# pengsongyou/openscene

Measured on NVIDIA B200. Metric: voxels/s MinkUNet34C fwd + 768-d cosine-sim, higher is better.
Workload: dtype bf16x3 (split fp32 operands, fp32 accumulate)

## Files before the change

### include/osb200.h

```cpp
#ifndef OSB200_H
#define OSB200_H

#include <stddef.h>
#include <stdint.h>

#ifdef __cplusplus
extern "C" {
#endif

#define OSB_VERSION 100

int         osb_version(void);
const char *osb_last_error(void);
int osb_device_info(int *sm_count, int *cc_major, int *cc_minor);
int64_t osb_launch_count(void);
int osb_measure_sm_mhz(float *mhz_dev, void *stream);

size_t osb_coordset_workspace_bytes(int64_t n);

int osb_coordset_build(const int32_t *coords, int64_t n, int32_t *coords_int, int32_t *perm, int32_t *inv_perm,
                       void *slots, int64_t cap, int32_t *status_host, void *ws, size_t ws_bytes, void *stream);

int osb_coordset_stride(const int32_t *coords_fine, int64_t n, int32_t new_ts, int32_t *coords_coarse,
                        int32_t *parent_of, int64_t *n_coarse_host, void *ws, size_t ws_bytes, void *stream);
// ... 6 lines not shown

int osb_kernel_map_build(const int32_t *coords_out, int64_t n_out, const void *slots_in, int64_t cap_in,
                         int32_t ks_x, int32_t ks_y, int32_t ks_z, int32_t step, int32_t *nbr,
                         int32_t *pairs_per_k, void *stream);

int osb_kernel_map_transpose(const int32_t *nbr, int64_t n_out, int32_t K, int32_t *nbr_t, int64_t n_in,
                             void *stream);

int osb_conv_fwd_f32(const float *in, int64_t ld_in, const int32_t *nbr, int64_t n_out, int32_t K,
                     const float *w, int32_t cin, int32_t cout, int32_t transpose_w, float *out, void *stream);

int osb_conv_wgrad_f32(const float *in, const int32_t *nbr, int64_t n_out, int32_t K, const float *gout,
                       int32_t cin, int32_t cout, float *gw, void *stream);

size_t osb_conv_wgrad_tc_workspace_bytes(int64_t n_out, int32_t K, int32_t cin, int32_t cout);
int osb_conv_wgrad_tc(const void *x_split, int32_t cin, int64_t n_in, const int32_t *nbr, int64_t n_out, int32_t K,
                      const void *gout_split, int32_t cout, float *gw, void *ws, size_t ws_bytes, void *stream);

size_t osb_conv_packed_weight_bytes(int32_t K, int32_t cin, int32_t cout);
size_t osb_conv_tc_workspace_bytes(int64_t n_out, int32_t K, int32_t cin, int32_t cout);
int osb_conv_pack_weights(const float *w, int32_t K, int32_t cin, int32_t cout, int32_t transpose_w,
                          void *wpack, void *stream);
int osb_conv_fwd_tc(const void *src0, int32_t c0, int64_t n_src0, const void *src1, int32_t c1, int64_t n_src1,
                    const int32_t *nbr, int64_t n_out, int32_t K, const void *wpack, int32_t cout,
                    const float *scale, const float *shift, const void *res, int32_t relu, void *out_split,
                    float *out_f32, const int32_t *out_row_map, void *ws, size_t ws_bytes, int32_t flags, void *stream);

int osb_convtr_fwd_tc(const void *src, int32_t cin, int64_t n_coarse, const int32_t *down_nbr, int32_t kvol, const void *wpack,
                      int32_t cout, const float *scale, const float *shift, int32_t relu, void *out_split, float *out_f32,
                      int32_t flags, void *stream);


size_t osb_conv_desc_bytes(void);
size_t osb_conv_weight_tiles_bytes(int32_t K, int32_t cin, int32_t cout);
int osb_conv_pack_weight_tiles(const float *w, int32_t K, int32_t cin, int32_t cout, int32_t transpose_w, void *wtiles,
                               void *stream);
int osb_conv_chain_grid(void);
size_t osb_conv_chain_workspace_bytes(int64_t n_out, int32_t K, int32_t cin, int32_t cout);
int osb_conv_desc_fill(void *desc_host, const void *src0, int32_t c0, const void *src1, int32_t c1, const int32_t *nbr,
                       int64_t n_out, int32_t K, const void *wtiles, int32_t cout, const float *scale, const float *shift,
                       const void *res, int32_t relu, void *out_split, float *out_f32, const int32_t *out_row_map,
                       const int32_t *cmap, int32_t cmap_cout, void *ws, size_t ws_bytes, int32_t barrier_before);
int osb_conv_chain_launch(const void *descs_host, int32_t n_layers, void *grid_barrier, int32_t flags, void *stream);

int osb_tuning_set(const char *name, int64_t value);

int osb_conv_stem_fused(const float *in, int32_t cin, const int32_t *coords, int64_t n, const void *slots,
                        int64_t cap, int32_t ks, int32_t step, const float *w, int32_t cout, const float *scale,
                        const float *shift, int32_t relu, void *out_split, float *out_f32, void *stream);

int osb_f32_to_split(const float *in, int64_t n, int32_t c, void *out_split, void *stream);
int osb_split_to_f32(const void *in_split, int64_t n, int32_t c, float *out, void *stream);

int osb_gather_rows_f32(const float *in, const int32_t *idx, int64_t n_out, int32_t c, float *out, void *stream);

int osb_match_scores(const void *feat, int32_t feat_is_f16, int64_t n_vox, int32_t c, const int64_t *inds_reverse,
                     int64_t n_pts, const void *text_f16, int32_t k_text, int32_t normalize, void *scores_f16,
                     int64_t *label, float *smax, void *stream);
int osb_match_ensemble(const float *feat3d, const void *feat2d_f16, int64_t n_vox, int32_t c,
                       const int64_t *inds_reverse, int64_t n_pts, const float *smax3d, const float *smax2d,
                       const void *text_f16, int32_t k_text, void *scores_f16, int64_t *label, void *feat_out_f16,
                       void *stream);

int osb_match_accumulate(const void *feat, int32_t feat_is_f16, const void *feat2_f16, const float *sel_a, const float *sel_b,
                         int64_t n_vox, int32_t c, const int64_t *inds_reverse, int64_t n_pts, const void *text_f16,
                         int32_t k_text, int32_t normalize, void *store_f16, int32_t first, int64_t *label, void *stream);
// ... 43 lines not shown
```

### openscene_b200/_cabi.py

```python
import ctypes
import os
from ctypes import c_char_p, c_double, c_int, c_int32, c_int64, c_size_t, c_void_p, POINTER

_HERE = os.path.dirname(os.path.abspath(__file__))
LIB_PATH = os.path.join(_HERE, 'libosb200.so')
_lib = None

P = c_void_p
I32, I64, SZ = c_int32, c_int64, c_size_t

SIGNATURES = {
    'osb_version': (c_int, []),
    'osb_last_error': (c_char_p, []),
    'osb_device_info': (c_int, [POINTER(c_int), POINTER(c_int), POINTER(c_int)]),
    'osb_launch_count': (I64, []),
    'osb_measure_sm_mhz': (c_int, [P, P]),
    'osb_coordset_workspace_bytes': (SZ, [I64]),
    'osb_coordset_build': (c_int, [P, I64, P, P, P, P, I64, POINTER(I32), P, SZ, P]),
    'osb_coordset_stride': (c_int, [P, I64, I32, P, P, POINTER(I64), P, SZ, P]),
    'osb_coordset_pyramid': (c_int, [P, I64, I32, P, P, P, P, I64, P, P, POINTER(I64), POINTER(I32), P, SZ, P]),
    'osb_hash_build': (c_int, [P, I64, P, I64, P]),
    'osb_kernel_map_build': (c_int, [P, I64, P, I64, I32, I32, I32, I32, P, P, P]),
    'osb_kernel_map_transpose': (c_int, [P, I64, I32, P, I64, P]),
    'osb_conv_fwd_f32': (c_int, [P, I64, P, I64, I32, P, I32, I32, I32, P, P]),
    'osb_conv_wgrad_f32': (c_int, [P, P, I64, I32, P, I32, I32, P, P]),
    'osb_conv_wgrad_tc_workspace_bytes': (SZ, [I64, I32, I32, I32]),
    'osb_conv_wgrad_tc': (c_int, [P, I32, I64, P, I64, I32, P, I32, P, P, SZ, P]),
    'osb_conv_packed_weight_bytes': (SZ, [I32, I32, I32]),
    'osb_conv_pack_weights': (c_int, [P, I32, I32, I32, I32, P, P]),
    'osb_conv_tc_workspace_bytes': (SZ, [I64, I32, I32, I32]),
    'osb_conv_fwd_tc': (c_int, [P, I32, I64, P, I32, I64, P, I64, I32, P, I32, P, P, P, I32, P, P, P, P, SZ, I32, P]),
    'osb_convtr_fwd_tc': (c_int, [P, I32, I64, P, I32, P, I32, P, P, I32, P, P, I32, P]),
    'osb_conv_desc_bytes': (SZ, []),
    'osb_conv_weight_tiles_bytes': (SZ, [I32, I32, I32]),
    'osb_conv_pack_weight_tiles': (c_int, [P, I32, I32, I32, I32, P, P]),
    'osb_conv_chain_grid': (c_int, []),
    'osb_conv_chain_workspace_bytes': (SZ, [I64, I32, I32, I32]),
    'osb_conv_desc_fill': (c_int, [P, P, I32, P, I32, P, I64, I32, P, I32, P, P, P, I32, P, P, P, P, I32, P, SZ, I32]),
    'osb_conv_chain_launch': (c_int, [P, I32, P, I32, P]),
    'osb_tuning_set': (c_int, [c_char_p, I64]),
    'osb_conv_stem_fused': (c_int, [P, I32, P, I64, P, I64, I32, I32, P, I32, P, P, I32, P, P, P]),
    'osb_f32_to_split': (c_int, [P, I64, I32, P, P]),
    'osb_split_to_f32': (c_int, [P, I64, I32, P, P]),
    'osb_gather_rows_f32': (c_int, [P, P, I64, I32, P, P]),
    'osb_match_scores': (c_int, [P, I32, I64, I32, P, I64, P, I32, I32, P, P, P, P]),
    'osb_match_ensemble': (c_int, [P, P, I64, I32, P, I64, P, P, P, I32, P, P, P, P]),
    'osb_match_accumulate': (c_int, [P, I32, P, P, P, I64, I32, P, I64, P, I32, I32, P, I32, P, P]),
    'osb_logits_accumulate': (c_int, [P, I64, I32, P, I64, P, I32, P, P, P]),
    'osb_folded_head_finish': (c_int, [P, I64, I32, I32, I32, P, P, P, P]),
    'osb_voxelize_workspace_bytes': (SZ, [I64]),
    'osb_voxelize': (c_int, [P, I32, I64, POINTER(c_double), P, P, P, POINTER(I64), POINTER(c_double), P, SZ, P]),
    'osb_occgrid_bytes': (SZ, [I32, I32]),
    'osb_occgrid_build': (c_int, [P, I64, I32, I32, I32, P, P, P]),
    'osb_kernel_map_build_grid': (c_int, [P, I64, P, I32, I32, I32, I32, I32, I32, I32, P, P, P]),
    'osb_conv_stem_fused_grid': (c_int, [P, I32, P, I64, P, I32, I32, I32, I32, I32, P, I32, P, P, I32, P, P, P]),
    'osb_fusion_workspace_bytes': (SZ, [I64, I32]),
    'osb_fusion_accumulate': (c_int, [P, I32, I64, P, P, P, P, I32, I32, I32, I32, I32, c_double, P, P, P, P, SZ, P]),
    'osb_fusion_finalize': (c_int, [P, P, I64, I32, P, P]),
    'osb_feature_remap_workspace_bytes': (SZ, [I64, I64]),
    'osb_feature_remap': (c_int, [P, I64, P, I64, P, I64, I32, I32, P, P, POINTER(I64), P, SZ, P]),
    'osb_confusion_accumulate': (c_int, [P, P, I32, I64, I32, I32, I32, P, P, P]),
    'osb_intersection_union': (c_int, [P, P, I32, I64, I32, I32, P, P]),
}


def lib():
# ... 41 lines not shown
```

### openscene_b200/csrc/conv_chain.cu

```cuda
#include "tc_ptx.cuh"
#include <algorithm>
#include <cstring>
#include <string>

namespace osb {

constexpr int CH_THREADS = 384;
constexpr int CH_M = 128;
constexpr int CH_A_BYTES = CH_M * 128;
constexpr int CH_STG_BYTES = 4 * 4096;
constexpr int CH_SS_FLOATS = 768;
constexpr int CH_MAX_SA = 12, CH_MAX_SB = 4;
constexpr int CH_W_EPI = 0;
constexpr int CH_W_B = 4;
constexpr int CH_W_MMA = 5;
constexpr int CH_W_A = 7;
constexpr int CH_A_WARPS = 5;
constexpr int CH_DESC_WORDS = 48;
constexpr int CH_MAX_LAYERS = 16;

struct __align__(16) ConvDesc {
  const uint8_t *src0, *src1;
  const int32_t *nbr;
  const uint8_t *wtiles;
  const float *scale, *shift;
  const uint8_t *res;
  uint8_t *out_split;
  float *out_f32;
  const int32_t *out_row_map;
  const int32_t *cmap;
  float *partial;
  int64_t n_out;
  int K, nb0, nb1;
  int cout, cout_pad, nt, n_ntiles;
  int relu, cmap_cout, nsplit, m_tiles;
  int nsub_max;
  int barrier_before;
  int stages_per_split;
  int pad[8];
};
static_assert(sizeof(ConvDesc) == CH_DESC_WORDS * 4, "ConvDesc layout");
struct ChainArgs { ConvDesc d[CH_MAX_LAYERS]; };

__device__ __forceinline__ void bulk_g2s(uint32_t dst, const void *src, uint32_t bytes, uint32_t bar) {
  asm volatile("cp.async.bulk.shared::cluster.global.mbarrier::complete_tx::bytes [%0], [%1], %2, [%3];"
               ::"r"(dst), "l"(src), "r"(bytes), "r"(bar) : "memory");
}
__device__ __forceinline__ void mbar_arrive(uint32_t bar) {
  asm volatile("mbarrier.arrive.shared::cta.b64 _, [%0];" ::"r"(bar) : "memory");
}
__device__ __forceinline__ uint32_t mbar_try(uint32_t bar, uint32_t parity) {
  uint32_t done;
  asm volatile(
      "{\n\t.reg .pred p;\n\t"
      "mbarrier.try_wait.parity.shared::cta.b64 p, [%1], %2;\n\t"
      "selp.u32 %0, 1, 0, p;\n\t}"
      : "=r"(done)
      : "r"(bar), "r"(parity)
      : "memory");
  return done;
}

__device__ long long *g_chain_report = nullptr;
__device__ __noinline__ void chain_stuck(uint32_t bar, uint32_t parity, int tag, uint32_t it) {
  long long *r = g_chain_report;
  if (r && it == (1u << 20) + 1) {
    long long *o = r + 1 + 4 * ((blockIdx.x * 16 + (threadIdx.x >> 5)) % 1024);
    o[0] = ((long long)blockIdx.x << 32) | (threadIdx.x >> 5); o[1] = bar; o[2] = parity; o[3] = tag;
    r[0] = 1;
    __threadfence_system();
  }
  if (it > (1u << 23) || !r) __trap();
}
__device__ __forceinline__ void chain_wait(uint32_t bar, uint32_t parity, int tag) {
  for (uint32_t it = 0;; ++it) {
// ... 15 lines not shown
    if (!done) {
      __nanosleep(sleep_ns);
      if (it > (1u << 24)) __trap();
    }
  }
}
__device__ __forceinline__ unsigned ld_acquire_u32(const unsigned *p) {
  unsigned v;
  asm volatile("ld.acquire.gpu.global.u32 %0, [%1];" : "=r"(v) : "l"(p) : "memory");
  return v;
}

__device__ __forceinline__ void grid_barrier(unsigned *gbar, unsigned &gen) {
  __syncthreads();
  if (threadIdx.x == 0) {
    __threadfence();
    const unsigned old = atomicAdd(gbar, 1u);
    if (old == gridDim.x - 1) {
      gbar[0] = 0;
      __threadfence();
      atomicAdd(gbar + 1, 1u);
    } else {
      unsigned it = 0;
      while (ld_acquire_u32(gbar + 1) == gen) {
        if (++it > (1u << 24)) __trap();
      }
    }
    __threadfence();
  }
  gen += 1;
  __syncthreads();
}

#define CH_PROF_BEGIN() const long long _t0 = prof ? clock64() : 0
#define CH_PROF_END(var) do { if (prof) var += clock64() - _t0; } while (0)

#define CH_KEEP(x) asm volatile("" : "+r"(x))

__device__ __forceinline__ void cp_async16_zfill(uint32_t dst, const void *src, uint32_t ignore) {
  asm volatile(
      "{\n\t.reg .pred p;\n\t"
      "setp.ne.b32 p, %2, 0;\n\t"
      "cp.async.cg.shared.global [%0], [%1], 16, p;\n\t}"
      ::"r"(dst), "l"(src), "r"(ignore)
      : "memory");
}

__global__ void __launch_bounds__(CH_THREADS, 1)
k_conv_chain(const __grid_constant__ ChainArgs args, int n_layers, unsigned *gbar, int sa, int sb, int bslot, int flags,
             long long *dbg_clock) {
  extern __shared__ uint8_t smem_raw[];
  const uint32_t raw_u32 = smem_u32(smem_raw);
  const uint32_t base_u32 = (raw_u32 + 1023u) & ~1023u;
  uint8_t *smem = smem_raw + (base_u32 - raw_u32);
  const uint32_t a_ring = base_u32;
  const uint32_t b_ring = a_ring + (uint32_t)sa * CH_A_BYTES;
  const uint32_t stg_u32 = b_ring + (uint32_t)sb * (uint32_t)bslot;
  uint32_t a_ring_k = a_ring, b_ring_k = b_ring;
  CH_KEEP(a_ring_k); CH_KEEP(b_ring_k);
  uint8_t *aux = smem + (stg_u32 - base_u32) + CH_STG_BYTES;
  float *s_ss = reinterpret_cast<float *>(aux);
  uint64_t *bars = reinterpret_cast<uint64_t *>(s_ss + 2 * CH_SS_FLOATS);
  uint32_t *s_misc = reinterpret_cast<uint32_t *>(bars + 40);

  const int tid = threadIdx.x, warp = tid >> 5, lane = tid & 31;
  if (flags & 1) asm volatile("griddepcontrol.launch_dependents;" ::: "memory");
  const bool prof = dbg_clock != nullptr;
  long long pw0 = 0, pw1 = 0, pw2 = 0, pt = 0;
  if (dbg_clock && tid == 0) dbg_clock[blockIdx.x * 32 + 0] = clock64();
  uint32_t fullA = smem_u32(bars), emptyA = fullA + 12 * 8, fullB = fullA + 24 * 8, emptyB = fullA + 28 * 8;
  uint32_t accFull = fullA + 32 * 8, accEmpty = fullA + 34 * 8;
  CH_KEEP(fullA); CH_KEEP(emptyA); CH_KEEP(fullB); CH_KEEP(emptyB); CH_KEEP(accFull); CH_KEEP(accEmpty);

  if (tid == 0) {
    for (int s = 0; s < sa; ++s) { mbar_init(fullA + 8 * s, 32); mbar_init(emptyA + 8 * s, 1); }
    for (int s = 0; s < sb; ++s) { mbar_init(fullB + 8 * s, 1); mbar_init(emptyB + 8 * s, 2); }
    for (int b = 0; b < 2; ++b) { mbar_init(accFull + 8 * b, 2); mbar_init(accEmpty + 8 * b, 4); }
    asm volatile("fence.mbarrier_init.release.cluster;" ::: "memory");
  }
  if (warp == CH_W_MMA) {
    asm volatile("tcgen05.alloc.cta_group::1.sync.aligned.shared::cta.b32 [%0], %1;" ::"r"(smem_u32(&s_misc[0])), "r"(512u));
    asm volatile("tcgen05.relinquish_alloc_permit.cta_group::1.sync.aligned;");
  }
  unsigned bar_gen = 0;
  if (tid == 0 && gbar) bar_gen = ld_acquire_u32(gbar + 1);
  asm volatile("tcgen05.fence::before_thread_sync;" ::: "memory");
  __syncthreads();
  asm volatile("tcgen05.fence::after_thread_sync;" ::: "memory");
  if (flags & 1) asm volatile("griddepcontrol.wait;" ::: "memory");
  const uint32_t tmem_base = s_misc[0];
  if (dbg_clock && tid == 0) dbg_clock[blockIdx.x * 32 + 1] = clock64();

  uint32_t a_slot = 0, a_phase = 0, b_slot = 0, b_phase = 0, n_item = 0;
  uint32_t g_slot = 0;
  uint32_t p_sl = warp >= CH_W_A ? (uint32_t)(warp - CH_W_A) : 0u, p_lapb = 0, p_par = 0;

  for (int L = 0; L < n_layers; ++L) {
    __syncthreads();
    const ConvDesc *s_desc = &args.d[L];
    const int d_K = s_desc->K, d_nb0 = s_desc->nb0, d_nb1 = s_desc->nb1, d_nt = s_desc->nt, d_n_ntiles = s_desc->n_ntiles;
    const int d_m_tiles = s_desc->m_tiles, d_nsplit = s_desc->nsplit, d_nsub_max = s_desc->nsub_max, d_sps = s_desc->stages_per_split;
    const int64_t d_n_out = s_desc->n_out;
    {
      const int nss = s_desc->cmap ? s_desc->cmap_cout : s_desc->cout;
      const float *sc = s_desc->scale, *sh = s_desc->shift;
      for (int c = tid; c < nss && c < CH_SS_FLOATS; c += CH_THREADS) {
        s_ss[c] = sc ? __ldg(sc + c) : 1.f;
        s_ss[CH_SS_FLOATS + c] = sh ? __ldg(sh + c) : 0.f;
      }
    }
    if (s_desc->barrier_before) {
      grid_barrier(gbar, bar_gen);
    } else {
      __syncthreads();
    }

    const int nb = d_nb0 + d_nb1;
    const int T = d_K * nb;
    const int64_t U = (int64_t)d_m_tiles * d_n_ntiles * d_nsplit;
    const int64_t u_begin = U * blockIdx.x / gridDim.x, u_end = U * (blockIdx.x + 1) / gridDim.x;
    const int per_z = d_m_tiles * d_n_ntiles;
    const uint32_t b_bytes = (uint32_t)d_nt * 128u;

#define CH_FOR_ITEMS()                                                                                         \
    for (int64_t u = u_begin, _n; u < u_end; u += _n)                                                          \
      if (const int z = (int)(u / per_z), r_ = (int)(u - (int64_t)z * per_z), nti = r_ / d_m_tiles,            \
          m = r_ - nti * d_m_tiles, nsub = (d_nsub_max == 2 && u + 1 < u_end && m + 1 < d_m_tiles) ? 2 : 1,    \
          t_begin = min(z * d_sps, T), t_end = min(t_begin + d_sps, T);                                        \
          (_n = nsub, true))

    const long long _role_t0 = prof ? clock64() : 0;
    if (warp == CH_W_B) {
      const uint8_t *wtiles = s_desc->wtiles;
      CH_FOR_ITEMS() {
        (void)m;
        for (int t = t_begin; t < t_end; ++t) {
          { CH_PROF_BEGIN(); mbar_wait_relaxed(emptyB + 8 * b_slot, b_phase ^ 1, 64); CH_PROF_END(pw0); }
          if (elect_one()) {
            const uint32_t fb = fullB + 8 * b_slot;
            if (flags & 0x200) {
              mbar_expect_tx(fb, 0u);
            } else {
              mbar_expect_tx(fb, b_bytes);
              bulk_g2s(b_ring_k + b_slot * (uint32_t)bslot, wtiles + ((int64_t)t * d_n_ntiles + nti) * b_bytes, b_bytes, fb);
            }
          }
          __syncwarp();
          if (++b_slot == (uint32_t)sb) { b_slot = 0; b_phase ^= 1; }
        }
      }
    } else if (warp == CH_W_MMA || warp == CH_W_MMA + 1) {
      const int mi = warp - CH_W_MMA;
      const uint32_t idesc = (1u << 4) | (1u << 7) | (1u << 10) | ((uint32_t)(d_nt >> 3) << 17) | ((uint32_t)(CH_M >> 4) << 24);
      CH_FOR_ITEMS() {
        (void)m; (void)nti;
        const uint32_t buf = n_item & 1u;
        const bool mine = mi < nsub;
        { CH_PROF_BEGIN(); mbar_wait(accEmpty + 8 * buf, ((n_item >> 1) & 1u) ^ 1u); CH_PROF_END(pw2); }
        asm volatile("tcgen05.fence::after_thread_sync;" ::: "memory");
        const uint32_t dcol = tmem_base + buf * 256u + (uint32_t)mi * 128u;
        for (int t = t_begin; t < t_end;) {
          const int nst = min(2, t_end - t);
          uint32_t sl[2], sph[2], bs[2], bph[2];
          {
            uint32_t as_ = a_slot + (uint32_t)mi, ap_ = a_phase, bs_ = b_slot, bp_ = b_phase;
            if (as_ >= (uint32_t)sa) { as_ -= (uint32_t)sa; ap_ ^= 1u; }
// ... 233 lines not shown
            }
            if (d_out_split) {
#pragma unroll
              for (int g = 0; g < 4; ++g) {
                __align__(16) __nv_bfloat16 hh[8], ll[8];
#pragma unroll
                for (int jj = 0; jj < 8; ++jj) split_bf16(y[g * 8 + jj], hh[jj], ll[jj]);
                sts128(my_line + ((g ^ sw) << 4), *reinterpret_cast<const uint4 *>(hh));
                sts128(my_line + (((4 + g) ^ sw) << 4), *reinterpret_cast<const uint4 *>(ll));
              }
              __syncwarp();
              flush_tile(d_out_split, (int64_t)out_c * 4, (int64_t)(oc0 >> 5) * 128, d_cmap != nullptr);
              __syncwarp();
            }
            if (d_out_f32) {
#pragma unroll
              for (int g = 0; g < 8; ++g)
                sts128(my_line + ((g ^ sw) << 4), make_uint4(__float_as_uint(y[4 * g]), __float_as_uint(y[4 * g + 1]),
                                                             __float_as_uint(y[4 * g + 2]), __float_as_uint(y[4 * g + 3])));
              __syncwarp();
              flush_tile(reinterpret_cast<uint8_t *>(d_out_f32), (int64_t)out_c * 4, (int64_t)oc0 * 4,
                         d_row_map != nullptr || d_cmap != nullptr);
              __syncwarp();
            }
          }
        }
        asm volatile("tcgen05.fence::before_thread_sync;" ::: "memory");
        __syncwarp();
        if (lane == 0) mbar_arrive(accEmpty + 8 * buf);
        ++n_item;
      }
    }
#undef CH_FOR_ITEMS
    if (prof) pt += clock64() - _role_t0;

    if (d_nsplit > 1) {
      grid_barrier(gbar, bar_gen);
      const ConvDesc &d = args.d[L];
      const int groups = d.cout / 8;
      const int64_t total = d.n_out * groups;
      for (int64_t e = (int64_t)blockIdx.x * CH_THREADS + tid; e < total; e += (int64_t)gridDim.x * CH_THREADS) {
        const int64_t o = e / groups;
        const int c0 = (int)(e - o * groups) * 8;
        float y[8] = {0.f, 0.f, 0.f, 0.f, 0.f, 0.f, 0.f, 0.f};
        for (int z = 0; z < d.nsplit; ++z) {
          const float4 *pp = reinterpret_cast<const float4 *>(d.partial + ((int64_t)z * d.n_out + o) * d.cout_pad + c0);
          const float4 a = __ldcg(pp), b = __ldcg(pp + 1);
          y[0] += a.x; y[1] += a.y; y[2] += a.z; y[3] += a.w; y[4] += b.x; y[5] += b.y; y[6] += b.z; y[7] += b.w;
        }
        if (d.scale) {
#pragma unroll
          for (int jj = 0; jj < 8; ++jj) y[jj] = fmaf(y[jj], s_ss[c0 + jj], s_ss[CH_SS_FLOATS + c0 + jj]);
        }
        const int64_t off = o * (int64_t)d.cout * 4 + split_off_hi(c0);
        if (d.res) {
          const uint4 hq = __ldcg(reinterpret_cast<const uint4 *>(d.res + off)), lq = __ldcg(reinterpret_cast<const uint4 *>(d.res + off + 64));
          const __nv_bfloat16 *hh = reinterpret_cast<const __nv_bfloat16 *>(&hq);
          const __nv_bfloat16 *ll = reinterpret_cast<const __nv_bfloat16 *>(&lq);
#pragma unroll
          for (int jj = 0; jj < 8; ++jj) y[jj] += join_bf16(hh[jj], ll[jj]);
        }
        if (d.relu) {
#pragma unroll
          for (int jj = 0; jj < 8; ++jj) y[jj] = fmaxf(y[jj], 0.f);
        }
        if (d.out_split) {
          __align__(16) __nv_bfloat16 hh[8], ll[8];
#pragma unroll
          for (int jj = 0; jj < 8; ++jj) split_bf16(y[jj], hh[jj], ll[jj]);
          *reinterpret_cast<uint4 *>(d.out_split + off) = *reinterpret_cast<const uint4 *>(hh);
          *reinterpret_cast<uint4 *>(d.out_split + off + 64) = *reinterpret_cast<const uint4 *>(ll);
        }
        if (d.out_f32) {
          const int64_t orow = d.out_row_map ? (int64_t)__ldg(d.out_row_map + o) : o;
          float4 *op = reinterpret_cast<float4 *>(d.out_f32 + orow * d.cout + c0);
          op[0] = make_float4(y[0], y[1], y[2], y[3]);
          op[1] = make_float4(y[4], y[5], y[6], y[7]);
        }
      }
    }
  }

  if (dbg_clock && tid == 0) dbg_clock[blockIdx.x * 32 + 2] = clock64();
  if (dbg_clock && lane == 0 && (warp == CH_W_B || warp == CH_W_MMA || warp == CH_W_MMA + 1 || warp == CH_W_A || warp == 0)) {
    const int base = warp == CH_W_B ? 4 : warp == CH_W_MMA ? 8 : warp == CH_W_MMA + 1 ? 12 : warp == CH_W_A ? 16 : 20;
    long long *o = dbg_clock + blockIdx.x * 32 + base;
    o[0] = pw0; o[1] = pw1; o[2] = pw2; o[3] = pt;
  }
  asm volatile("tcgen05.fence::before_thread_sync;" ::: "memory");
  __syncthreads();
  if (warp == CH_W_MMA) asm volatile("tcgen05.dealloc.cta_group::1.sync.aligned.b32 %0, %1;" ::"r"(tmem_base), "r"(512u));
}

__global__ void k_pack_weight_tiles(const float *__restrict__ w, int K, int cin, int cout, int cout_pad, int nt, int transpose_w,
                                    uint8_t *__restrict__ wt) {
  const int nb = cin / 32, n_ntiles = cout_pad / nt;
  const int64_t total = (int64_t)K * cout_pad * cin;
  for (int64_t e = (int64_t)blockIdx.x * blockDim.x + threadIdx.x; e < total; e += (int64_t)gridDim.x * blockDim.x) {
    const int c = (int)(e % cin);
    const int64_t kn = e / cin;
    const int ng = (int)(kn % cout_pad), k = (int)(kn / cout_pad);
    float v = 0.f;
    if (ng < cout) v = transpose_w ? w[((int64_t)k * cout + ng) * cin + c] : w[((int64_t)k * cin + c) * cout + ng];
    __nv_bfloat16 hi, lo;
    split_bf16(v, hi, lo);
    const int cb = c >> 5, ci = c & 31, nti = ng / nt, n = ng - nti * nt;
    uint8_t *tile = wt + ((((int64_t)k * nb + cb) * n_ntiles) + nti) * (int64_t)nt * 128;
    const int jh = ci >> 3, el = ci & 7;
    *reinterpret_cast<__nv_bfloat16 *>(tile + n * 128 + (((jh) ^ (n & 7)) << 4) + el * 2) = hi;
    *reinterpret_cast<__nv_bfloat16 *>(tile + n * 128 + (((4 + jh) ^ (n & 7)) << 4) + el * 2) = lo;
  }
}

}

namespace osb { bool conv_tc_tuning(const char *name, int64_t v); }
using namespace osb;

static inline int chain_cout_pad(int cout) { return cout <= 256 ? (cout + 15) / 16 * 16 : (cout + 255) / 256 * 256; }
static inline int chain_nt(int cout) { const int cp = chain_cout_pad(cout); return cp <= 256 ? cp : 256; }

extern "C" {

size_t osb_conv_desc_bytes(void) { return sizeof(ConvDesc); }

size_t osb_conv_weight_tiles_bytes(int32_t K, int32_t cin, int32_t cout) { return (size_t)K * chain_cout_pad(cout) * cin * 4; }

int osb_conv_pack_weight_tiles(const float *w, int32_t K, int32_t cin, int32_t cout, int32_t transpose_w, void *wtiles, void *stream_) {
  cudaStream_t stream = (cudaStream_t)stream_;
  OSB_CHECK(K >= 1 && cin % 32 == 0 && cin > 0 && cout > 0, "osb_conv_pack_weight_tiles: cin (%d) must be a multiple of 32", cin);
  const int cp = chain_cout_pad(cout), nt = chain_nt(cout);
  const int64_t total = (int64_t)K * cp * cin;
  const unsigned grid = (unsigned)std::min<int64_t>(ceil_div(total, 256), 148 * 32);
  k_pack_weight_tiles<<<grid, 256, 0, stream>>>(w, K, cin, cout, cp, nt, transpose_w, (uint8_t *)wtiles);
  OSB_LAUNCH_CHECK();
  return 0;
}

static int chain_nsplit(int64_t n_out, int K, int cin, int cout, int grid_ctas, int force, int nsub_knob) {
  const int cp = chain_cout_pad(cout), nt = chain_nt(cout);
  const int64_t tiles = ceil_div(n_out, CH_M) * (cp / nt);
  const int T = K * (cin / 32);
  const int cap = std::max(1, std::min(32, T));
  if (force > 0) return std::min(force, cap);
  const bool pairs = nt <= 128 && nsub_knob >= 2;
  const int base = (int)std::max<int64_t>(1, std::min<int64_t>(grid_ctas / tiles, cap));
  auto cost = [&](int ns, bool &ok) {
    const int sps = (T + ns - 1) / ns;
    ok = (T + sps - 1) / sps == ns;
    const int64_t upc = ceil_div(tiles * ns, (int64_t)grid_ctas);
    const double per = pairs ? (double)(upc / 2) * 0.75 + (double)(upc % 2) * 0.6 : (double)upc * 0.6 * 1.6;
    double us = per * sps + 4.0;
    if (ns > 1) {
      const double partial_bytes = (double)ns * (double)n_out * cp * 4.0;
      if (partial_bytes > 64e6) ok = false;
      us += 10.0 + 2.0 * partial_bytes / 5e6;
    }
    return us;
  };
  bool ok = true;
  double best = cost(base, ok);
  int best_ns = base;
  for (int ns = base + 1; ns <= cap; ++ns) {
    const double us = cost(ns, ok);
    if (ok && us < best - std::max(0.5, 0.08 * best)) { best = us; best_ns = ns; }
  }
  return best_ns;
}

static int g_chain_force_split = 0;
static int g_chain_nsub = 2;
static int g_chain_grid = 0;
static int g_chain_sa = 0, g_chain_sb = 0;
static long long *g_chain_dbg_clock = nullptr;
static int g_chain_dbg_skip = 0;

int osb_tuning_set(const char *name, int64_t value) {
  const std::string n(name ? name : "");
  if (n == "chain_force_split") g_chain_force_split = (int)value;
  else if (n == "chain_nsub") g_chain_nsub = (int)value;
  else if (n == "chain_grid") g_chain_grid = (int)value;
  else if (n == "chain_sa") g_chain_sa = (int)value;
  else if (n == "chain_sb") g_chain_sb = (int)value;
  else if (n == "chain_dbg_clock") g_chain_dbg_clock = (long long *)(intptr_t)value;
  else if (n == "chain_dbg_skip") g_chain_dbg_skip = (int)value;
  else if (n == "chain_report") {
    long long *ptr = (long long *)(intptr_t)value;
    OSB_CUDA(cudaMemcpyToSymbol(g_chain_report, &ptr, sizeof(ptr)));
  }
  else { OSB_CHECK(conv_tc_tuning(n.c_str(), value), "osb_tuning_set: unknown knob '%s'", n.c_str()); }
  return 0;
}

int osb_conv_chain_grid(void) {
  if (g_chain_grid > 0) return g_chain_grid;
  int dev = 0, sms = 148;
  if (cudaGetDevice(&dev) == cudaSuccess) cudaDeviceGetAttribute(&sms, cudaDevAttrMultiProcessorCount, dev);
  return sms;
}

size_t osb_conv_chain_workspace_bytes(int64_t n_out, int32_t K, int32_t cin, int32_t cout) {
  if (n_out <= 0 || K < 1 || cin < 32 || cout <= 0) return 0;
  const int ns = chain_nsplit(n_out, K, cin, cout, osb_conv_chain_grid(), g_chain_force_split, g_chain_nsub);
  return ns > 1 ? (size_t)ns * n_out * chain_cout_pad(cout) * sizeof(float) : 0;
}

int osb_conv_desc_fill(void *desc_host, const void *src0, int32_t c0, const void *src1, int32_t c1, const int32_t *nbr, int64_t n_out,
                       int32_t K, const void *wtiles, int32_t cout, const float *scale, const float *shift, const void *res,
                       int32_t relu, void *out_split, float *out_f32, const int32_t *out_row_map, const int32_t *cmap,
                       int32_t cmap_cout, void *ws, size_t ws_bytes, int32_t barrier_before) {
  OSB_CHECK(desc_host != nullptr, "osb_conv_desc_fill: no descriptor");
  OSB_CHECK(src0 && c0 > 0 && c0 % 32 == 0 && c1 >= 0 && c1 % 32 == 0, "osb_conv_desc_fill: channel counts must be multiples of 32 (c0=%d c1=%d)", c0, c1);
  OSB_CHECK((c1 == 0) == (src1 == nullptr), "osb_conv_desc_fill: src1 / c1 mismatch");
  OSB_CHECK(K >= 1 && K <= 32, "osb_conv_desc_fill: K=%d not supported (<= 32)", K);
  OSB_CHECK(nbr != nullptr || K == 1, "osb_conv_desc_fill: identity map needs K == 1");
  OSB_CHECK(n_out > 0 && n_out < (1ll << 31), "osb_conv_desc_fill: bad row count");
  OSB_CHECK(cout % 32 == 0 && cout > 0, "osb_conv_desc_fill: cout (%d) must be a multiple of 32", cout);
// ... 1 lines not shown
  OSB_CHECK((scale == nullptr) == (shift == nullptr), "osb_conv_desc_fill: scale and shift go together");
  OSB_CHECK(cmap == nullptr || (cmap_cout > 0 && cmap_cout % 32 == 0 && cout % cmap_cout == 0 && res == nullptr),
            "osb_conv_desc_fill: bad dense-transpose arguments");
  OSB_CHECK((cmap ? cmap_cout : cout) <= CH_SS_FLOATS, "osb_conv_desc_fill: more than %d output channels per row", CH_SS_FLOATS);
  ConvDesc d{};
  const int cin = c0 + c1;
  d.src0 = (const uint8_t *)src0; d.src1 = (const uint8_t *)src1; d.nbr = nbr; d.wtiles = (const uint8_t *)wtiles;
  d.scale = scale; d.shift = shift; d.res = (const uint8_t *)res; d.out_split = (uint8_t *)out_split; d.out_f32 = out_f32;
  d.out_row_map = out_row_map; d.cmap = cmap; d.n_out = n_out; d.K = K; d.nb0 = c0 / 32; d.nb1 = c1 / 32;
  d.cout = cout; d.cout_pad = chain_cout_pad(cout); d.nt = chain_nt(cout); d.n_ntiles = d.cout_pad / d.nt;
  d.relu = relu; d.cmap_cout = cmap_cout; d.m_tiles = (int)ceil_div(n_out, CH_M);
  d.nsub_max = (d.nt <= 128 && g_chain_nsub >= 2) ? 2 : 1;
  d.barrier_before = barrier_before ? 1 : 0;
  d.nsplit = cmap ? 1 : chain_nsplit(n_out, K, cin, cout, osb_conv_chain_grid(), g_chain_force_split, g_chain_nsub);
  const int T = K * (cin / 32);
  d.stages_per_split = (T + d.nsplit - 1) / d.nsplit;
  d.nsplit = (T + d.stages_per_split - 1) / d.stages_per_split;
  d.partial = nullptr;
  if (d.nsplit > 1) {
    const size_t need = (size_t)d.nsplit * n_out * d.cout_pad * sizeof(float);
    OSB_CHECK(ws != nullptr && ws_bytes >= need, "osb_conv_desc_fill: workspace of %zu bytes required (got %zu)", need, ws_bytes);
    d.partial = (float *)ws;
  }
  memcpy(desc_host, &d, sizeof(d));
  return 0;
}

int osb_conv_chain_launch(const void *descs_host, int32_t n_layers, void *grid_barrier_dev, int32_t flags, void *stream_) {
  cudaStream_t stream = (cudaStream_t)stream_;
  OSB_CHECK(descs_host && n_layers >= 1, "osb_conv_chain_launch: bad arguments");
  const ConvDesc *h = (const ConvDesc *)descs_host;
  for (int i = 0; i < n_layers; ++i) {
    OSB_CHECK(i > 0 || !h[i].barrier_before, "osb_conv_chain_launch: the first layer of a launch cannot ask for a barrier");
    OSB_CHECK(i == 0 || h[i].barrier_before || h[i].nsplit == 1 || h[i - 1].nsplit == 1 || h[i].partial != h[i - 1].partial,
              "osb_conv_chain_launch: layers %d and %d share a split workspace without a barrier between them", i - 1, i);
  }
  OSB_SMEM_ATTR_ONCE(k_conv_chain, 227 * 1024);
  const int grid = osb_conv_chain_grid();
  for (int l0 = 0; l0 < n_layers; l0 += CH_MAX_LAYERS) {
    const int cnt = std::min(CH_MAX_LAYERS, n_layers - l0);
    ChainArgs args;
    memcpy(args.d, h + l0, sizeof(ConvDesc) * cnt);
    args.d[0].barrier_before = 0;
    int nt_max = 0, need_bar = 0;
    for (int i = 0; i < cnt; ++i) {
      nt_max = std::max(nt_max, args.d[i].nt);
      need_bar |= (args.d[i].barrier_before || args.d[i].nsplit > 1);
    }
    OSB_CHECK(!need_bar || grid_barrier_dev != nullptr, "osb_conv_chain_launch: this chain needs the grid-barrier words");
    const int bslot = nt_max * 128;
    const int fixed = 1024 + CH_STG_BYTES + 2 * CH_SS_FLOATS * 4 + 40 * 8 + 64;
    int sb = g_chain_sb > 0 ? g_chain_sb : (bslot >= 32768 ? 2 : 3);
    sb = std::min(sb, CH_MAX_SB);
    int sa = (227 * 1024 - fixed - sb * bslot) / CH_A_BYTES;
    if (g_chain_sa > 0) sa = std::min(sa, g_chain_sa);
    sa = std::min(sa, CH_MAX_SA);
    sa &= ~1;
    OSB_CHECK(sa >= 4, "osb_conv_chain_launch: shared memory does not hold four row slots");
    const size_t smem_bytes = (size_t)sa * CH_A_BYTES + (size_t)sb * bslot + fixed;
    cudaLaunchAttribute attr[1];
    attr[0].id = cudaLaunchAttributeProgrammaticStreamSerialization;
    attr[0].val.programmaticStreamSerializationAllowed = 1;
    cudaLaunchConfig_t cfg{};
    cfg.gridDim = dim3((unsigned)grid); cfg.blockDim = dim3(CH_THREADS); cfg.dynamicSmemBytes = smem_bytes; cfg.stream = stream;
    cfg.attrs = attr; cfg.numAttrs = (flags & 1) ? 1 : 0;
    OSB_CUDA(cudaLaunchKernelEx(&cfg, k_conv_chain, args, (int)cnt, (unsigned *)grid_barrier_dev, sa, sb, bslot,
                                (int)((flags & 1) | (g_chain_dbg_skip << 8)), g_chain_dbg_clock));
    OSB_LAUNCH_CHECK();
  }
  return 0;
}

}
```

### openscene_b200/tc.py

```python
import ctypes
import weakref

import torch

from . import _cabi as C


def to_split(x):
    x = x.contiguous()
    n, c = x.shape
    out = torch.empty((n, 4 * c), dtype=torch.uint8, device=x.device)
    C.call('osb_f32_to_split', C.ptr(x), n, c, C.ptr(out), C.stream_ptr())
    return out


def from_split(xs, c):
    n = xs.shape[0]
    out = torch.empty((n, c), dtype=torch.float32, device=xs.device)
    C.call('osb_split_to_f32', C.ptr(xs), n, c, C.ptr(out), C.stream_ptr())
    return out


def pack_weights(w3, transpose_w=False):
    w3 = w3.detach().contiguous().float()
# ... 55 lines not shown
    if hit is None:
        hit = ent[3][k] = pack_weights(w3, transpose_w)
    return hit


def conv_stem(x, coords, slots, cap, ks, step, w3, scale=None, shift=None, relu=False, out_split=True, out_f32=False):
    n, cin = x.shape
    cout = w3.shape[2]
    os_ = torch.empty((n, 4 * cout), dtype=torch.uint8, device=x.device) if out_split else None
    of_ = torch.empty((n, cout), dtype=torch.float32, device=x.device) if out_f32 else None
    C.call('osb_conv_stem_fused', C.ptr(x.contiguous()), cin, C.ptr(coords), n, C.ptr(slots), cap, ks, step,
           C.ptr(w3.contiguous()), cout, C.ptr(scale), C.ptr(shift), int(relu), C.ptr(os_), C.ptr(of_), C.stream_ptr())
    return os_, of_


def pack_weight_tiles(w3, transpose_w=False):
    w3 = w3.detach().contiguous().float()
    K = w3.shape[0]
    cin, cout = (w3.shape[2], w3.shape[1]) if transpose_w else (w3.shape[1], w3.shape[2])
    nbytes = C.lib().osb_conv_weight_tiles_bytes(K, cin, cout)
    out = torch.empty(nbytes, dtype=torch.uint8, device=w3.device)
    C.call('osb_conv_pack_weight_tiles', C.ptr(w3), K, cin, cout, int(transpose_w), C.ptr(out), C.stream_ptr())
    return out


class ConvChain:

    def __init__(self, device, max_layers=160):
        self.device = torch.device(device)
        self.dbytes = C.lib().osb_conv_desc_bytes()
        self.max_layers = max_layers
        self.host = torch.zeros(max_layers * self.dbytes, dtype=torch.uint8)
        with torch.cuda.device(self.device):
            self.gbar = torch.zeros(4, dtype=torch.int32, device=self.device)
        self.host_a, self.gbar_a = self.host.data_ptr(), self.gbar.data_ptr()
        self._fill = C.lib().osb_conv_desc_fill
        self.begin()

    def begin(self):
        self.n = 0
        self.groups = []
        self._g0 = 0

    def add(self, src0, c0, src1, c1, nbr, n_out, K, wtiles, cout, scale=0, shift=0, res=0, relu=0, out_split=0, out_f32=0,
            row_map=0, cmap=0, cmap_cout=0, ws=0, ws_bytes=0, barrier_before=0):
        if self.n >= self.max_layers:
            raise RuntimeError("ConvChain: too many layers")
        rc = self._fill(self.host_a + self.n * self.dbytes, src0, c0, src1 or None, c1, nbr or None, n_out, K, wtiles, cout,
                        scale or None, shift or None, res or None, int(relu), out_split or None, out_f32 or None,
                        row_map or None, cmap or None, cmap_cout, ws or None, ws_bytes,
                        int(bool(barrier_before) and self.n > self._g0))
        if rc:
            C.check(rc, 'osb_conv_desc_fill')
        self.n += 1

    def cut(self):
        if self.n > self._g0:
            self.groups.append((self._g0, self.n - self._g0))
            self._g0 = self.n

    def run(self, flags=0, stream=None):
        self.cut()
        stream = stream if stream is not None else torch.cuda.current_stream().cuda_stream
        fn = C.lib().osb_conv_chain_launch
        for (g0, cnt) in self.groups:
            rc = fn(self.host_a + g0 * self.dbytes, cnt, self.gbar_a, flags, stream)
            if rc:
# ... 50 lines not shown
```

Before: 41.73 million.

## Replace grid barrier before split-K reduction with per-tile counters and add L2 weight prefetch

For split-K layers, each CTA now bumps a per-output-tile arrival counter and waits only on the tiles it reduces, instead of waiting at a grid-wide barrier before the reduction. The reduction work is also split across the split index, and counters reset themselves through atomicInc wrap-around. The B-loader warp additionally prefetches the next layer's weight tiles into L2, and the chain can hold up to 48 layers, with a 16-layer template kept for short launches. In exchange the sync buffer is larger, spin-waits can trap, and phase-timing debug hooks are added.

```diff
diff --git a/include/osb200.h b/include/osb200.h
--- a/include/osb200.h
+++ b/include/osb200.h
@@ -62,6 +62,8 @@
 
 
 size_t osb_conv_desc_bytes(void);
+size_t osb_conv_chain_sync_bytes(void);
+int osb_conv_chain_max_layers(void);
 size_t osb_conv_weight_tiles_bytes(int32_t K, int32_t cin, int32_t cout);
 int osb_conv_pack_weight_tiles(const float *w, int32_t K, int32_t cin, int32_t cout, int32_t transpose_w, void *wtiles,
                                void *stream);
diff --git a/openscene_b200/_cabi.py b/openscene_b200/_cabi.py
--- a/openscene_b200/_cabi.py
+++ b/openscene_b200/_cabi.py
@@ -32,6 +32,8 @@
     'osb_conv_fwd_tc': (c_int, [P, I32, I64, P, I32, I64, P, I64, I32, P, I32, P, P, P, I32, P, P, P, P, SZ, I32, P]),
     'osb_convtr_fwd_tc': (c_int, [P, I32, I64, P, I32, P, I32, P, P, I32, P, P, I32, P]),
     'osb_conv_desc_bytes': (SZ, []),
+    'osb_conv_chain_sync_bytes': (SZ, []),
+    'osb_conv_chain_max_layers': (c_int, []),
     'osb_conv_weight_tiles_bytes': (SZ, [I32, I32, I32]),
     'osb_conv_pack_weight_tiles': (c_int, [P, I32, I32, I32, I32, P, P]),
     'osb_conv_chain_grid': (c_int, []),
diff --git a/openscene_b200/csrc/conv_chain.cu b/openscene_b200/csrc/conv_chain.cu
--- a/openscene_b200/csrc/conv_chain.cu
+++ b/openscene_b200/csrc/conv_chain.cu
@@ -17,7 +17,12 @@
 constexpr int CH_W_A = 7;
 constexpr int CH_A_WARPS = 5;
 constexpr int CH_DESC_WORDS = 48;
-constexpr int CH_MAX_LAYERS = 16;
+constexpr int CH_MAX_LAYERS = 48;
+constexpr int CH_SHORT_LAYERS = 16;
+constexpr int CH_SYNC_HDR = 4;
+constexpr int CH_SYNC_TILES = 1024;
+constexpr int CH_PHASES = 8;
+constexpr int CH_PHASE_LAYERS = 256;
 
 struct __align__(16) ConvDesc {
   const uint8_t *src0, *src1;
@@ -37,10 +42,11 @@
   int nsub_max;
   int barrier_before;
   int stages_per_split;
-  int pad[8];
+  int tile_sync;
+  int pad[7];
 };
 static_assert(sizeof(ConvDesc) == CH_DESC_WORDS * 4, "ConvDesc layout");
-struct ChainArgs { ConvDesc d[CH_MAX_LAYERS]; };
+template <int NL> struct ChainArgs { ConvDesc d[NL]; };
 
 __device__ __forceinline__ void bulk_g2s(uint32_t dst, const void *src, uint32_t bytes, uint32_t bar) {
   asm volatile("cp.async.bulk.shared::cluster.global.mbarrier::complete_tx::bytes [%0], [%1], %2, [%3];"
@@ -122,6 +128,27 @@
   __syncthreads();
 }
 
+__device__ __forceinline__ void tile_arrive(unsigned *c) {
+  asm volatile("red.release.gpu.global.add.u32 [%0], 1;" ::"l"(c) : "memory");
+}
+__device__ __forceinline__ void tile_wait(const unsigned *c, unsigned target) {
+  unsigned it = 0;
+  while (ld_acquire_u32(c) < target) {
+    if (++it > (1u << 24)) __trap();
+  }
+}
+__device__ __forceinline__ long long global_ns() {
+  long long t;
+  asm volatile("mov.u64 %0, %%globaltimer;" : "=l"(t));
+  return t;
+}
+__device__ __forceinline__ void prefetch_l2(const void *p, uint32_t bytes) {
+  asm volatile("cp.async.bulk.prefetch.L2.global [%0], %1;" ::"l"(p), "r"(bytes) : "memory");
+}
+
+__device__ __forceinline__ int prof_slot(int warp) {
+  return warp == CH_W_B ? 4 : warp == CH_W_MMA ? 8 : warp == CH_W_MMA + 1 ? 12 : warp == CH_W_A ? 16 : warp == 0 ? 20 : -1;
+}
 #define CH_PROF_BEGIN() const long long _t0 = prof ? clock64() : 0
 #define CH_PROF_END(var) do { if (prof) var += clock64() - _t0; } while (0)
 
@@ -136,9 +163,58 @@
       : "memory");
 }
 
+__device__ __noinline__ void chain_reduce(const ConvDesc *dp, const float *s_ss, int64_t row0, int c_begin, int groups,
+                                         int64_t e0, int64_t e_end, int64_t step) {
+  const ConvDesc &d = *dp;
+  for (int64_t e = e0; e < e_end; e += step) {
+    const int64_t o = row0 + e / groups;
+    const int c0 = c_begin + (int)(e % groups) * 4;
+    float y[4] = {0.f, 0.f, 0.f, 0.f};
+    const float *pz = d.partial + o * d.cout_pad + c0;
+    const int64_t zstride = d.n_out * d.cout_pad;
+    for (int z0 = 0; z0 < d.nsplit; z0 += 4) {
+      float4 a[4];
+#pragma unroll
+      for (int j = 0; j < 4; ++j)
+        if (z0 + j < d.nsplit) a[j] = __ldcg(reinterpret_cast<const float4 *>(pz + (int64_t)(z0 + j) * zstride));
+#pragma unroll
+      for (int j = 0; j < 4; ++j)
+        if (z0 + j < d.nsplit) { y[0] += a[j].x; y[1] += a[j].y; y[2] += a[j].z; y[3] += a[j].w; }
+    }
+    if (d.scale) {
+#pragma unroll
+      for (int jj = 0; jj < 4; ++jj) y[jj] = fmaf(y[jj], s_ss[c0 + jj], s_ss[CH_SS_FLOATS + c0 + jj]);
+    }
+    const int64_t off = o * (int64_t)d.cout * 4 + split_off_hi(c0);
+    if (d.res) {
+      const uint2 hq = __ldcg(reinterpret_cast<const uint2 *>(d.res + off)), lq = __ldcg(reinterpret_cast<const uint2 *>(d.res + off + 64));
+      const __nv_bfloat16 *hh = reinterpret_cast<const __nv_bfloat16 *>(&hq);
+      const __nv_bfloat16 *ll = reinterpret_cast<const __nv_bfloat16 *>(&lq);
+#pragma unroll
+      for (int jj = 0; jj < 4; ++jj) y[jj] += join_bf16(hh[jj], ll[jj]);
+    }
+    if (d.relu) {
+#pragma unroll
+      for (int jj = 0; jj < 4; ++jj) y[jj] = fmaxf(y[jj], 0.f);
+    }
+    if (d.out_split) {
+      __align__(8) __nv_bfloat16 hh[4], ll[4];
+#pragma unroll
+      for (int jj = 0; jj < 4; ++jj) split_bf16(y[jj], hh[jj], ll[jj]);
+      *reinterpret_cast<uint2 *>(d.out_split + off) = *reinterpret_cast<const uint2 *>(hh);
+      *reinterpret_cast<uint2 *>(d.out_split + off + 64) = *reinterpret_cast<const uint2 *>(ll);
+    }
+    if (d.out_f32) {
+      const int64_t orow = d.out_row_map ? (int64_t)__ldg(d.out_row_map + o) : o;
+      *reinterpret_cast<float4 *>(d.out_f32 + orow * d.cout + c0) = make_float4(y[0], y[1], y[2], y[3]);
+    }
+  }
+}
+
+template <int NL>
 __global__ void __launch_bounds__(CH_THREADS, 1)
-k_conv_chain(const __grid_constant__ ChainArgs args, int n_layers, unsigned *gbar, int sa, int sb, int bslot, int flags,
-             long long *dbg_clock) {
+k_conv_chain(const __grid_constant__ ChainArgs<NL> args, int n_layers, unsigned *gbar, int sa, int sb, int bslot, int flags,
+             long long *dbg_clock, long long *dbg_phase) {
   extern __shared__ uint8_t smem_raw[];
   const uint32_t raw_u32 = smem_u32(smem_raw);
   const uint32_t base_u32 = (raw_u32 + 1023u) & ~1023u;
@@ -156,8 +232,9 @@
   const int tid = threadIdx.x, warp = tid >> 5, lane = tid & 31;
   if (flags & 1) asm volatile("griddepcontrol.launch_dependents;" ::: "memory");
   const bool prof = dbg_clock != nullptr;
-  long long pw0 = 0, pw1 = 0, pw2 = 0, pt = 0;
+  long long pw0 = 0, pw1 = 0, pw2 = 0;
   if (dbg_clock && tid == 0) dbg_clock[blockIdx.x * 32 + 0] = clock64();
+  if (dbg_clock && lane == 0 && prof_slot(warp) >= 0) dbg_clock[blockIdx.x * 32 + prof_slot(warp) + 3] = 0;
   uint32_t fullA = smem_u32(bars), emptyA = fullA + 12 * 8, fullB = fullA + 24 * 8, emptyB = fullA + 28 * 8;
   uint32_t accFull = fullA + 32 * 8, accEmpty = fullA + 34 * 8;
   CH_KEEP(fullA); CH_KEEP(emptyA); CH_KEEP(fullB); CH_KEEP(emptyB); CH_KEEP(accFull); CH_KEEP(accEmpty);
@@ -185,8 +262,11 @@
   uint32_t g_slot = 0;
   uint32_t p_sl = warp >= CH_W_A ? (uint32_t)(warp - CH_W_A) : 0u, p_lapb = 0, p_par = 0;
 
+#define CH_PHASE(k) do { if (dbg_phase && tid == 0) dbg_phase[((int64_t)L * gridDim.x + blockIdx.x) * CH_PHASES + (k)] = global_ns(); } while (0)
+
   for (int L = 0; L < n_layers; ++L) {
     __syncthreads();
+    CH_PHASE(0);
     const ConvDesc *s_desc = &args.d[L];
     const int d_K = s_desc->K, d_nb0 = s_desc->nb0, d_nb1 = s_desc->nb1, d_nt = s_desc->nt, d_n_ntiles = s_desc->n_ntiles;
     const int d_m_tiles = s_desc->m_tiles, d_nsplit = s_desc->nsplit, d_nsub_max = s_desc->nsub_max, d_sps = s_desc->stages_per_split;
@@ -204,6 +284,7 @@
     } else {
       __syncthreads();
     }
+    CH_PHASE(1);
 
     const int nb = d_nb0 + d_nb1;
     const int T = d_K * nb;
@@ -222,6 +303,26 @@
     const long long _role_t0 = prof ? clock64() : 0;
     if (warp == CH_W_B) {
       const uint8_t *wtiles = s_desc->wtiles;
+      if (n_layers > 1 && !(flags & 0x200) && lane == 0) {
+        auto prefetch_layer = [&](const ConvDesc *pd) {
+          const int T_ = pd->K * (pd->nb0 + pd->nb1), sps = pd->stages_per_split, mt = pd->m_tiles, ntn = pd->n_ntiles;
+          const int64_t per = (int64_t)mt * ntn, U_ = per * pd->nsplit;
+          const int64_t ub = U_ * blockIdx.x / gridDim.x, ue = U_ * (blockIdx.x + 1) / gridDim.x;
+          const uint32_t bb = (uint32_t)pd->nt * 128u;
+          int64_t prev = -1;
+          for (int64_t u = ub; u < ue; ++u) {
+            const int z = (int)(u / per), nti = (int)(u - z * per) / mt;
+            const int64_t key = (int64_t)z * ntn + nti;
+            if (key == prev) continue;
+            prev = key;
+            const int tb = min(z * sps, T_), te = min(tb + sps, T_);
+            for (int t = tb; t < te; ++t) prefetch_l2(pd->wtiles + ((int64_t)t * ntn + nti) * bb, bb);
+          }
+        };
+        if (L == 0) prefetch_layer(&args.d[0]);
+        if (L + 1 < n_layers) prefetch_layer(&args.d[L + 1]);
+      }
+      __syncwarp();
       CH_FOR_ITEMS() {
         (void)m;
         for (int t = t_begin; t < t_end; ++t) {
@@ -521,60 +622,55 @@
       }
     }
 #undef CH_FOR_ITEMS
-    if (prof) pt += clock64() - _role_t0;
-
+    if (prof && lane == 0 && prof_slot(warp) >= 0)
+      dbg_clock[blockIdx.x * 32 + prof_slot(warp) + 3] += clock64() - _role_t0;
+
+    if (dbg_phase && d_nsplit == 1) { __syncthreads(); CH_PHASE(2); }
     if (d_nsplit > 1) {
-      grid_barrier(gbar, bar_gen);
       const ConvDesc &d = args.d[L];
-      const int groups = d.cout / 8;
-      const int64_t total = d.n_out * groups;
-      for (int64_t e = (int64_t)blockIdx.x * CH_THREADS + tid; e < total; e += (int64_t)gridDim.x * CH_THREADS) {
-        const int64_t o = e / groups;
-        const int c0 = (int)(e - o * groups) * 8;
-        float y[8] = {0.f, 0.f, 0.f, 0.f, 0.f, 0.f, 0.f, 0.f};
-        for (int z = 0; z < d.nsplit; ++z) {
-          const float4 *pp = reinterpret_cast<const float4 *>(d.partial + ((int64_t)z * d.n_out + o) * d.cout_pad + c0);
-          const float4 a = __ldcg(pp), b = __ldcg(pp + 1);
-          y[0] += a.x; y[1] += a.y; y[2] += a.z; y[3] += a.w; y[4] += b.x; y[5] += b.y; y[6] += b.z; y[7] += b.w;
+      if (d.tile_sync) {
+        unsigned *cnt = gbar + CH_SYNC_HDR + L * CH_SYNC_TILES;
+        int ns = d.nsplit, mt = d.m_tiles, tnt = d.nt, bx = (int)blockIdx.x;
+        CH_KEEP(ns); CH_KEEP(mt); CH_KEEP(tnt); CH_KEEP(bx);
+        const int tiles = mt * d.n_ntiles;
+        const int ub = (int)((int64_t)tiles * ns * bx / gridDim.x), ue = (int)((int64_t)tiles * ns * (bx + 1) / gridDim.x);
+        __syncthreads();
+        CH_PHASE(2);
+        if (tid == 0) {
+          __threadfence();
+          for (int u = ub; u < ue; ++u) tile_arrive(cnt + u % tiles);
         }
-        if (d.scale) {
-#pragma unroll
-          for (int jj = 0; jj < 8; ++jj) y[jj] = fmaf(y[jj], s_ss[c0 + jj], s_ss[CH_SS_FLOATS + c0 + jj]);
+        CH_PHASE(3);
+        for (int u = ub; u < ue; ++u) {
+          const int z = u / tiles, p = u - z * tiles, nti = p / mt, m = p - nti * mt;
+          if (tid == 0) tile_wait(cnt + p, (unsigned)ns);
+          __syncthreads();
+          if (u == ub) CH_PHASE(4);
+          const int row0 = m * CH_M;
+          const int rows = (int)min((int64_t)CH_M, d.n_out - row0);
+          const int groups = min(tnt, d.cout - nti * tnt) / 4;
+          const int total = rows * groups;
+          chain_reduce(&d, s_ss, row0, nti * tnt, groups, total * z / ns + tid, total * (z + 1) / ns, CH_THREADS);
+          __syncthreads();
+          if (tid == 0) atomicInc(cnt + p, 2u * (unsigned)ns - 1u);
         }
-        const int64_t off = o * (int64_t)d.cout * 4 + split_off_hi(c0);
-        if (d.res) {
-          const uint4 hq = __ldcg(reinterpret_cast<const uint4 *>(d.res + off)), lq = __ldcg(reinterpret_cast<const uint4 *>(d.res + off + 64));
-          const __nv_bfloat16 *hh = reinterpret_cast<const __nv_bfloat16 *>(&hq);
-          const __nv_bfloat16 *ll = reinterpret_cast<const __nv_bfloat16 *>(&lq);
-#pragma unroll
-          for (int jj = 0; jj < 8; ++jj) y[jj] += join_bf16(hh[jj], ll[jj]);
-        }
-        if (d.relu) {
-#pragma unroll
-          for (int jj = 0; jj < 8; ++jj) y[jj] = fmaxf(y[jj], 0.f);
-        }
-        if (d.out_split) {
-          __align__(16) __nv_bfloat16 hh[8], ll[8];
-#pragma unroll
-          for (int jj = 0; jj < 8; ++jj) split_bf16(y[jj], hh[jj], ll[jj]);
-          *reinterpret_cast<uint4 *>(d.out_split + off) = *reinterpret_cast<const uint4 *>(hh);
-          *reinterpret_cast<uint4 *>(d.out_split + off + 64) = *reinterpret_cast<const uint4 *>(ll);
-        }
-        if (d.out_f32) {
-          const int64_t orow = d.out_row_map ? (int64_t)__ldg(d.out_row_map + o) : o;
-          float4 *op = reinterpret_cast<float4 *>(d.out_f32 + orow * d.cout + c0);
-          op[0] = make_float4(y[0], y[1], y[2], y[3]);
-          op[1] = make_float4(y[4], y[5], y[6], y[7]);
-        }
+        CH_PHASE(5);
+      } else {
+        if (dbg_phase) { __syncthreads(); CH_PHASE(2); }
+        grid_barrier(gbar, bar_gen);
+        CH_PHASE(4);
+        chain_reduce(&d, s_ss, 0, 0, d.cout / 4, (int64_t)blockIdx.x * CH_THREADS + tid, d.n_out * (d.cout / 4),
+                     (int64_t)gridDim.x * CH_THREADS);
+        CH_PHASE(5);
       }
     }
   }
+#undef CH_PHASE
 
   if (dbg_clock && tid == 0) dbg_clock[blockIdx.x * 32 + 2] = clock64();
-  if (dbg_clock && lane == 0 && (warp == CH_W_B || warp == CH_W_MMA || warp == CH_W_MMA + 1 || warp == CH_W_A || warp == 0)) {
-    const int base = warp == CH_W_B ? 4 : warp == CH_W_MMA ? 8 : warp == CH_W_MMA + 1 ? 12 : warp == CH_W_A ? 16 : 20;
-    long long *o = dbg_clock + blockIdx.x * 32 + base;
-    o[0] = pw0; o[1] = pw1; o[2] = pw2; o[3] = pt;
+  if (dbg_clock && lane == 0 && prof_slot(warp) >= 0) {
+    long long *o = dbg_clock + blockIdx.x * 32 + prof_slot(warp);
+    o[0] = pw0; o[1] = pw1; o[2] = pw2;
   }
   asm volatile("tcgen05.fence::before_thread_sync;" ::: "memory");
   __syncthreads();
@@ -612,6 +708,10 @@
 extern "C" {
 
 size_t osb_conv_desc_bytes(void) { return sizeof(ConvDesc); }
+
+size_t osb_conv_chain_sync_bytes(void) { return (size_t)(CH_SYNC_HDR + CH_MAX_LAYERS * CH_SYNC_TILES) * sizeof(uint32_t); }
+
+int osb_conv_chain_max_layers(void) { return CH_MAX_LAYERS; }
 
 size_t osb_conv_weight_tiles_bytes(int32_t K, int32_t cin, int32_t cout) { return (size_t)K * chain_cout_pad(cout) * cin * 4; }
 
@@ -661,7 +761,10 @@
 static int g_chain_nsub = 2;
 static int g_chain_grid = 0;
 static int g_chain_sa = 0, g_chain_sb = 0;
+static int g_chain_sync = 1;
 static long long *g_chain_dbg_clock = nullptr;
+static long long *g_chain_dbg_phase = nullptr;
+static int g_chain_phase_next = 0;
 static int g_chain_dbg_skip = 0;
 
 int osb_tuning_set(const char *name, int64_t value) {
@@ -671,7 +774,9 @@
   else if (n == "chain_grid") g_chain_grid = (int)value;
   else if (n == "chain_sa") g_chain_sa = (int)value;
   else if (n == "chain_sb") g_chain_sb = (int)value;
+  else if (n == "chain_sync") g_chain_sync = value ? 1 : 0;
   else if (n == "chain_dbg_clock") g_chain_dbg_clock = (long long *)(intptr_t)value;
+  else if (n == "chain_dbg_phase") { g_chain_dbg_phase = (long long *)(intptr_t)value; g_chain_phase_next = 0; }
   else if (n == "chain_dbg_skip") g_chain_dbg_skip = (int)value;
   else if (n == "chain_report") {
     long long *ptr = (long long *)(intptr_t)value;
@@ -739,22 +844,32 @@
   const ConvDesc *h = (const ConvDesc *)descs_host;
   for (int i = 0; i < n_layers; ++i) {
     OSB_CHECK(i > 0 || !h[i].barrier_before, "osb_conv_chain_launch: the first layer of a launch cannot ask for a barrier");
-    OSB_CHECK(i == 0 || h[i].barrier_before || h[i].nsplit == 1 || h[i - 1].nsplit == 1 || h[i].partial != h[i - 1].partial,
-              "osb_conv_chain_launch: layers %d and %d share a split workspace without a barrier between them", i - 1, i);
-  }
-  OSB_SMEM_ATTR_ONCE(k_conv_chain, 227 * 1024);
+    if (h[i].nsplit > 1)
+      for (int j = i - 1; j >= 0 && !h[j + 1].barrier_before; --j)
+        OSB_CHECK(h[j].nsplit == 1 || h[j].partial != h[i].partial,
+                  "osb_conv_chain_launch: layers %d and %d share a split workspace without a barrier between them", j, i);
+  }
+  OSB_SMEM_ATTR_ONCE(k_conv_chain<CH_SHORT_LAYERS>, 227 * 1024);
+  OSB_SMEM_ATTR_ONCE(k_conv_chain<CH_MAX_LAYERS>, 227 * 1024);
   const int grid = osb_conv_chain_grid();
   for (int l0 = 0; l0 < n_layers; l0 += CH_MAX_LAYERS) {
     const int cnt = std::min(CH_MAX_LAYERS, n_layers - l0);
-    ChainArgs args;
+    ChainArgs<CH_MAX_LAYERS> args;
     memcpy(args.d, h + l0, sizeof(ConvDesc) * cnt);
     args.d[0].barrier_before = 0;
     int nt_max = 0, need_bar = 0;
     for (int i = 0; i < cnt; ++i) {
-      nt_max = std::max(nt_max, args.d[i].nt);
-      need_bar |= (args.d[i].barrier_before || args.d[i].nsplit > 1);
-    }
-    OSB_CHECK(!need_bar || grid_barrier_dev != nullptr, "osb_conv_chain_launch: this chain needs the grid-barrier words");
+      ConvDesc &d = args.d[i];
+      nt_max = std::max(nt_max, d.nt);
+      need_bar |= (d.barrier_before || d.nsplit > 1);
+      d.tile_sync = (g_chain_sync && d.nsplit > 1 && (int64_t)d.m_tiles * d.n_ntiles <= CH_SYNC_TILES) ? 1 : 0;
+    }
+    OSB_CHECK(!need_bar || grid_barrier_dev != nullptr, "osb_conv_chain_launch: this chain needs the sync buffer");
+    long long *phase = nullptr;
+    if (g_chain_dbg_phase && g_chain_phase_next + cnt <= CH_PHASE_LAYERS) {
+      phase = g_chain_dbg_phase + (int64_t)g_chain_phase_next * grid * CH_PHASES;
+      g_chain_phase_next += cnt;
+    }
     const int bslot = nt_max * 128;
     const int fixed = 1024 + CH_STG_BYTES + 2 * CH_SS_FLOATS * 4 + 40 * 8 + 64;
     int sb = g_chain_sb > 0 ? g_chain_sb : (bslot >= 32768 ? 2 : 3);
@@ -771,8 +886,16 @@
     cudaLaunchConfig_t cfg{};
     cfg.gridDim = dim3((unsigned)grid); cfg.blockDim = dim3(CH_THREADS); cfg.dynamicSmemBytes = smem_bytes; cfg.stream = stream;
     cfg.attrs = attr; cfg.numAttrs = (flags & 1) ? 1 : 0;
-    OSB_CUDA(cudaLaunchKernelEx(&cfg, k_conv_chain, args, (int)cnt, (unsigned *)grid_barrier_dev, sa, sb, bslot,
-                                (int)((flags & 1) | (g_chain_dbg_skip << 8)), g_chain_dbg_clock));
+    const int kflags = (int)((flags & 1) | (g_chain_dbg_skip << 8));
+    if (cnt <= CH_SHORT_LAYERS) {
+      ChainArgs<CH_SHORT_LAYERS> short_args;
+      memcpy(short_args.d, args.d, sizeof(ConvDesc) * cnt);
+      OSB_CUDA(cudaLaunchKernelEx(&cfg, k_conv_chain<CH_SHORT_LAYERS>, short_args, (int)cnt, (unsigned *)grid_barrier_dev, sa, sb,
+                                  bslot, kflags, g_chain_dbg_clock, phase));
+    } else {
+      OSB_CUDA(cudaLaunchKernelEx(&cfg, k_conv_chain<CH_MAX_LAYERS>, args, (int)cnt, (unsigned *)grid_barrier_dev, sa, sb, bslot,
+                                  kflags, g_chain_dbg_clock, phase));
+    }
     OSB_LAUNCH_CHECK();
   }
   return 0;
diff --git a/openscene_b200/tc.py b/openscene_b200/tc.py
--- a/openscene_b200/tc.py
+++ b/openscene_b200/tc.py
@@ -111,7 +111,8 @@
         self.max_layers = max_layers
         self.host = torch.zeros(max_layers * self.dbytes, dtype=torch.uint8)
         with torch.cuda.device(self.device):
-            self.gbar = torch.zeros(4, dtype=torch.int32, device=self.device)
+            nsync = C.lib().osb_conv_chain_sync_bytes() // 4
+            self.gbar = torch.zeros(nsync, dtype=torch.int32, device=self.device)
         self.host_a, self.gbar_a = self.host.data_ptr(), self.gbar.data_ptr()
         self._fill = C.lib().osb_conv_desc_fill
         self.begin()
```

Result: no change. 41.53 million (median of 6 runs) (-0.5%).
